# agnusmaximus/DistributedMNIST

Hardware: AMD Instinct MI355X
Metric: images/sec (whole node), MNIST CNN sync-SGD (higher is better)
Workload: dtype bf16; 1 GPU; model=lenet, global_batch=1024, parallelism=dp1, mode=full_sync, mode_requested=full_sync, grad_dtype=fp32

## Files before the change

csrc/bindings.cpp:

```cpp

#include <torch/extension.h>
#include <ATen/hip/HIPContext.h>
#include <hip/hip_runtime.h>

#include "kernels.h"

namespace {

#define CHECK_BF16(t) TORCH_CHECK((t).scalar_type() == at::kBFloat16, #t " must be bf16")
#define CHECK_F32(t) TORCH_CHECK((t).scalar_type() == at::kFloat, #t " must be fp32")
#define CHECK_CONTIG(t) TORCH_CHECK((t).is_contiguous(), #t " must be contiguous")
#define CHECK_CUDA(t) TORCH_CHECK((t).is_cuda(), #t " must be on GPU")

const unsigned short* bf16_ptr(const torch::Tensor& t) {
  return reinterpret_cast<const unsigned short*>(t.data_ptr());
}
unsigned short* bf16_mut(torch::Tensor& t) {
  return reinterpret_cast<unsigned short*>(t.data_ptr());
}

hipStream_t cur_stream() {
  return at::hip::getCurrentHIPStream().stream();
}

int cdiv(int a, int b) { return (a + b - 1) / b; }

int pick_splitk(int mtiles, int ntiles, int ksteps) {
  int tiles = mtiles * ntiles;
  if (tiles >= 256 || ksteps <= 1) return 1;
  int want = std::min(ksteps, std::max(1, 512 / tiles));
  return want;
}

int dw_tr_level() {
  static int v = [] {
    const char* e = getenv("DMNIST_DW_TR");
    return e ? atoi(e) : 1;
  }();
  return v;
}
bool dw_tr_enabled() { return dw_tr_level() != 0; }

torch::Tensor linear_act_fwd_impl(torch::Tensor x, torch::Tensor w,
                                  torch::Tensor b, bool relu, double p_keep,
                                  int64_t seed, int64_t offset,
                                  const long* offset_dev,
                                  const c10::optional<torch::Tensor>& wT) {
  CHECK_CUDA(x); CHECK_BF16(x); CHECK_CONTIG(x);
  CHECK_BF16(w); CHECK_CONTIG(w);
  CHECK_F32(b); CHECK_CONTIG(b);
  int M = x.size(0), K = x.size(1), N = w.size(1);
  TORCH_CHECK(w.size(0) == K, "w/x shape mismatch");
  auto y = torch::empty({M, N}, x.options());
  GemmParams p{};
  p.A = bf16_ptr(x);
  p.bias = b.data_ptr<float>();
  p.C = y.data_ptr(); p.amax = nullptr;
  p.M = M; p.N = N; p.K = K;
  p.lda = K; p.ldc = N;
  p.splitk = 1;
  p.p_keep = (float)p_keep; p.seed = (uint64_t)seed; p.offset = (uint64_t)offset;
  p.offset_dev = offset_dev;
  bool drop = p_keep < 1.0;
  TORCH_CHECK(!drop || relu, "dropout path requires relu epilogue");
  int g128 = cdiv(M, 128) * cdiv(N, 128);
  bool big = g128 >= 512;
  if (const char* e = getenv("DMNIST_FC_TILE")) big = atoi(e) >= 128;
  auto s = cur_stream();
  bool bt = wT.has_value() && wT->defined();
  int tiles64 = cdiv(M, 64) * cdiv(N, 64);
  int ksteps = cdiv(K, 64);
  if (!big && tiles64 < 256 && ksteps >= 16 &&
      !getenv("DMNIST_FC_NOSPLIT")) {
    int sk = std::min(ksteps, std::max(2, 512 / tiles64));
    auto acc = torch::empty({(int64_t)sk, (int64_t)M, (int64_t)N},
                            x.options().dtype(at::kFloat));
    p.C = acc.data_ptr();
    p.splitk = sk;
    if (bt) {
      CHECK_BF16((*wT)); CHECK_CONTIG((*wT));
      TORCH_CHECK(wT->size(0) == N && wT->size(1) == K, "wT shape mismatch");
      p.B = bf16_ptr(*wT); p.ldb = K;
      gemm_fwd_slices_64_bt(p, s);
    } else {
      p.B = bf16_ptr(w); p.ldb = N;
      gemm_fwd_slices_64(p, s);
    }
    launch_fwd_epilogue(acc.data_ptr<float>(), b.data_ptr<float>(),
                        bf16_mut(y), M, N, sk, relu ? 1 : 0, (float)p_keep,
                        (uint64_t)seed, (uint64_t)offset, offset_dev, s);
    return y;
  }
  if (bt) {
    CHECK_BF16((*wT)); CHECK_CONTIG((*wT));
    TORCH_CHECK(wT->size(0) == N && wT->size(1) == K, "wT shape mismatch");
    p.B = bf16_ptr(*wT); p.ldb = K;
    if (drop) (big ? gemm_fwd_drop_128_bt : gemm_fwd_drop_64_bt)(p, s);
    else if (relu) (big ? gemm_fwd_relu_128_bt : gemm_fwd_relu_64_bt)(p, s);
    else (big ? gemm_fwd_bias_128_bt : gemm_fwd_bias_64_bt)(p, s);
  } else {
    p.B = bf16_ptr(w); p.ldb = N;
    if (drop) (big ? gemm_fwd_drop_128 : gemm_fwd_drop_64)(p, s);
    else if (relu) (big ? gemm_fwd_relu_128 : gemm_fwd_relu_64)(p, s);
    else (big ? gemm_fwd_bias_128 : gemm_fwd_bias_64)(p, s);
  }
  return y;
}

torch::Tensor linear_act_fwd(torch::Tensor x, torch::Tensor w, torch::Tensor b,
                             bool relu, double p_keep, int64_t seed,
                             int64_t offset,
                             c10::optional<torch::Tensor> wT) {
  return linear_act_fwd_impl(x, w, b, relu, p_keep, seed, offset, nullptr, wT);
}

torch::Tensor linear_act_fwd_dev(torch::Tensor x, torch::Tensor w,
                                 torch::Tensor b, bool relu, double p_keep,
                                 int64_t seed, torch::Tensor offset_dev,
                                 c10::optional<torch::Tensor> wT) {
  TORCH_CHECK(offset_dev.scalar_type() == at::kLong && offset_dev.is_cuda(),
              "offset_dev must be a cuda int64 tensor");
  return linear_act_fwd_impl(x, w, b, relu, p_keep, seed, 0,
                             offset_dev.data_ptr<long>(), wT);
}

std::vector<torch::Tensor> linear_act_bwd_impl(torch::Tensor dy, torch::Tensor x,
                                               torch::Tensor w, torch::Tensor y,
                                               bool relu, double p_keep,
                                               bool need_dx,
                                               torch::Tensor dw, torch::Tensor db) {
  CHECK_CUDA(dy); CHECK_BF16(dy); CHECK_CONTIG(dy);
  CHECK_BF16(x); CHECK_CONTIG(x);
  CHECK_BF16(w); CHECK_CONTIG(w);
  int B = x.size(0), K = x.size(1), N = w.size(1);
  auto s = cur_stream();
  if (!db.defined())
    db = torch::zeros({N}, x.options().dtype(at::kFloat));
  CHECK_F32(db); CHECK_CONTIG(db);
  torch::Tensor dyeff;
  bool mask = relu || p_keep < 1.0;
  if (mask) {
    dyeff = torch::empty_like(dy);
    launch_relu_drop_bwd(bf16_ptr(dy), bf16_ptr(y), bf16_mut(dyeff),
                         db.data_ptr<float>(), B, N,
                         (float)(1.0 / p_keep), 1, s);
  } else {
    dyeff = dy;
    launch_relu_drop_bwd(bf16_ptr(dy), bf16_ptr(y), bf16_mut(dyeff),
                         db.data_ptr<float>(), B, N, 1.0f, 0, s);
  }
  if (!dw.defined())
    dw = torch::zeros({K, N}, x.options().dtype(at::kFloat));
  CHECK_F32(dw); CHECK_CONTIG(dw);
  {
    GemmParams p{};
    p.A = bf16_ptr(x); p.B = bf16_ptr(dyeff);
    p.C = dw.data_ptr();
    p.M = K; p.N = N; p.K = B;
    p.lda = K;
    p.ldb = N; p.ldc = N;
    if (dw_tr_enabled() && K % 8 == 0 && N % 64 == 0) {
      int bn = (N % 128 == 0) ? 128 : 64;
      p.splitk = pick_splitk(cdiv(K, 128), cdiv(N, bn), cdiv(B, 32));
      (bn == 128 ? gemm_dw_tr_128 : gemm_dw_tr_64)(p, s);
    } else {
      bool big = cdiv(K, 128) * cdiv(N, 128) >= 128;
      int bm = big ? 128 : 64;
      p.splitk = pick_splitk(cdiv(K, bm), cdiv(N, bm), cdiv(B, 32));
      (big ? gemm_dw_128 : gemm_dw_64)(p, s);
    }
  }
  torch::Tensor dx;
  if (need_dx) {
    dx = torch::empty({B, K}, x.options());
    GemmParams p{};
    p.A = bf16_ptr(dyeff); p.B = bf16_ptr(w);
    p.C = dx.data_ptr();
    p.M = B; p.N = K; p.K = N;
    p.lda = N; p.ldb = N; p.ldc = K;
    p.splitk = 1;
    bool big = cdiv(B, 128) * cdiv(K, 128) >= 128;
    (big ? gemm_dx_128 : gemm_dx_64)(p, s);
  } else {
    dx = torch::empty({0}, x.options());
  }
  return {dx, dw, db};
}

std::vector<torch::Tensor> linear_act_bwd(torch::Tensor dy, torch::Tensor x,
                                          torch::Tensor w, torch::Tensor y,
                                          bool relu, double p_keep,
                                          bool need_dx) {
  return linear_act_bwd_impl(dy, x, w, y, relu, p_keep, need_dx,
                             torch::Tensor(), torch::Tensor());
}

torch::Tensor linear_act_bwd_into(torch::Tensor dy, torch::Tensor x,
                                  torch::Tensor w, torch::Tensor y,
                                  bool relu, double p_keep, bool need_dx,
                                  torch::Tensor dw_out, torch::Tensor db_out) {
  auto r = linear_act_bwd_impl(dy, x, w, y, relu, p_keep, need_dx,
                               dw_out.view({x.size(1), w.size(1)}), db_out);
  return r[0];
}

std::vector<torch::Tensor> conv_pool_fwd(torch::Tensor x, torch::Tensor w,
                                         torch::Tensor b,
                                         c10::optional<torch::Tensor> wT) {
  CHECK_CUDA(x); CHECK_BF16(x); CHECK_CONTIG(x);
  CHECK_BF16(w); CHECK_CONTIG(w);
  CHECK_F32(b); CHECK_CONTIG(b);
  int NB = x.size(0), H = x.size(1), W = x.size(2), Cin = x.size(3);
  TORCH_CHECK(w.dim() == 4 && w.size(0) == 5 && w.size(1) == 5 &&
              w.size(2) == Cin, "conv weight must be [5,5,Cin,Cout]");
  int Cout = w.size(3);
  int Ho = H / 2, Wo = W / 2;
  auto y = torch::empty({NB, Ho, Wo, Cout}, x.options());
  auto amax = torch::empty({NB, Ho, Wo, Cout}, x.options().dtype(at::kByte));
  GemmParams p{};
  p.A = bf16_ptr(x); p.B = bf16_ptr(w);
  p.bias = b.data_ptr<float>();
  p.C = y.data_ptr(); p.amax = amax.data_ptr<uint8_t>();
  p.M = NB * Ho * Wo * 4; p.N = Cout; p.K = 25 * Cin;
  p.ldb = Cout; p.ldc = Cout;
  p.splitk = 1;
  p.CB = NB; p.CH = H; p.CW = W; p.CHo = Ho; p.CWo = Wo;
  p.Cin = Cin; p.Cout = Cout;
  auto s = cur_stream();
  if (Cin == 1 && conv1_mfma_supported(H, W, Cin, Cout) &&
      conv1_mfma_enabled() &&
      reinterpret_cast<uintptr_t>(x.data_ptr()) % 8 == 0) {
    launch_conv1_mfma_fwd(bf16_ptr(x), bf16_ptr(w), b.data_ptr<float>(),
                          bf16_mut(y), amax.data_ptr<uint8_t>(), NB, s);
  } else if (Cin == 1) {
    launch_conv1_direct_fwd(bf16_ptr(x), bf16_ptr(w), b.data_ptr<float>(),
                            bf16_mut(y), amax.data_ptr<uint8_t>(), NB, H, W,
                            Cout, s);
  } else if (conv_slab_supported(H, W, Cin, Cout)) {
    launch_conv_fwd_slab(bf16_ptr(x), bf16_ptr(w), b.data_ptr<float>(),
                         bf16_mut(y), amax.data_ptr<uint8_t>(), NB, H, W,
                         Cin, Cout, s);
  } else {
    TORCH_CHECK(Cin % 8 == 0, "conv requires Cin==1 or Cin%8==0");
    if (wT.has_value() && wT->defined()) {
      CHECK_BF16((*wT)); CHECK_CONTIG((*wT));
      p.B = bf16_ptr(*wT); p.ldb = 25 * Cin;
      conv_fwd_pool_bt(p, s);
    } else {
      conv_fwd_pool(p, s);
    }
  }
  return {y, amax};
}

std::vector<torch::Tensor> conv_pool_bwd_impl(torch::Tensor dy, torch::Tensor x,
                                              torch::Tensor w, torch::Tensor y,
                                              torch::Tensor amax, bool need_dx,
                                              torch::Tensor dw, torch::Tensor db) {
  CHECK_CUDA(dy); CHECK_BF16(dy); CHECK_CONTIG(dy);
  CHECK_BF16(x); CHECK_CONTIG(x); CHECK_BF16(w); CHECK_CONTIG(w);
  int NB = x.size(0), H = x.size(1), W = x.size(2), Cin = x.size(3);
  int Cout = w.size(3);
  int Ho = H / 2, Wo = W / 2;
  auto s = cur_stream();
  auto dact = torch::empty({NB, H, W, Cout}, x.options());
  if (!db.defined())
    db = torch::zeros({Cout}, x.options().dtype(at::kFloat));
  CHECK_F32(db); CHECK_CONTIG(db);
  launch_pool_bwd_scatter(bf16_ptr(dy), bf16_ptr(y),
                          amax.data_ptr<uint8_t>(), bf16_mut(dact),
                          db.data_ptr<float>(), NB * Ho * Wo, Cout, H, W, Wo,
                          s);
  if (!dw.defined())
    dw = torch::zeros({5, 5, Cin, Cout}, x.options().dtype(at::kFloat));
  CHECK_F32(dw); CHECK_CONTIG(dw);
  {
    GemmParams p{};
    p.A = bf16_ptr(x); p.B = bf16_ptr(dact);
    p.C = dw.data_ptr();
    p.M = 25 * Cin; p.N = Cout; p.K = NB * H * W;
    p.ldb = Cout; p.ldc = Cout;
    p.CB = NB; p.CH = H; p.CW = W; p.Cin = Cin; p.Cout = Cout;
    if (Cin == 1 && H <= 28 && W <= 28 && Cout <= 32 &&
        !getenv("DMNIST_DW1_SLAB")) {
      launch_conv1_dw_direct(bf16_ptr(x), bf16_ptr(dact),
                             dw.data_ptr<float>(), NB, H, W, Cout, s);
    } else if (Cin == 1 && conv1_slab_supported(H, W, Cin, Cout)) {
      launch_conv1_dw_slab(bf16_ptr(x), bf16_ptr(dact), dw.data_ptr<float>(),
                           NB, H, W, Cout, s);
    } else if (Cin == 1) {
      p.splitk = std::min(cdiv(p.K, 64), 2048);
      conv1_dw_gemm(p, s);
    } else if (conv_slab_supported(H, W, Cin, Cout) &&
               ((dw_tr_level() == 0 && NB >= 2048) || getenv("DMNIST_DW_G"))) {
      launch_conv_dw_slab(bf16_ptr(x), bf16_ptr(dact), dw.data_ptr<float>(),
                          NB, H, W, Cin, Cout, s);
    } else {
      int tiles = cdiv(p.M, 128) * cdiv(p.N, 64);
      int want = p.K <= 262144 ? 1024 : 2048;
      if (const char* e = getenv("DMNIST_DW_BLOCKS")) want = atoi(e);
      p.splitk = std::min(cdiv(p.K, 64), std::max(1, want / tiles));
      if (dw_tr_enabled() && Cin % 8 == 0 && Cout % 64 == 0)
        conv_dw_tr(p, s);
      else
        conv_dw_gemm(p, s);
    }
  }
  torch::Tensor dx;
  if (need_dx && conv_slab_supported(H, W, Cin, Cout)) {
    dx = torch::empty({NB, H, W, Cin}, x.options());
    launch_conv_dx_slab(bf16_ptr(dact), bf16_ptr(w), bf16_mut(dx), NB, H, W,
                        Cin, Cout, s);
  } else if (need_dx) {
    TORCH_CHECK(Cout % 32 == 0, "conv_dx requires Cout%32==0");
    dx = torch::empty({NB, H, W, Cin}, x.options());
    GemmParams p{};
    p.A = bf16_ptr(dact); p.B = bf16_ptr(w);
    p.C = dx.data_ptr();
    p.M = NB * H * W; p.N = Cin; p.K = 25 * Cout;
    p.ldc = Cin;
    p.CB = NB; p.CH = H; p.CW = W; p.Cin = Cin; p.Cout = Cout;
    p.splitk = 1;
    conv_dx_gemm(p, s);
  } else {
    dx = torch::empty({0}, x.options());
  }
  return {dx, dw, db};
}

std::vector<torch::Tensor> conv_pool_bwd(torch::Tensor dy, torch::Tensor x,
                                         torch::Tensor w, torch::Tensor y,
                                         torch::Tensor amax, bool need_dx) {
  return conv_pool_bwd_impl(dy, x, w, y, amax, need_dx, torch::Tensor(),
                            torch::Tensor());
}

torch::Tensor conv_pool_bwd_into(torch::Tensor dy, torch::Tensor x,
                                 torch::Tensor w, torch::Tensor y,
                                 torch::Tensor amax, bool need_dx,
                                 torch::Tensor dw_out, torch::Tensor db_out) {
  auto r = conv_pool_bwd_impl(dy, x, w, y, amax, need_dx,
                              dw_out.view_as(w), db_out);
  return r[0];
}

torch::Tensor mask_db(torch::Tensor dy, torch::Tensor y, bool relu,
                      double p_keep, torch::Tensor db_out) {
  CHECK_CUDA(dy); CHECK_BF16(dy); CHECK_CONTIG(dy);
  CHECK_F32(db_out); CHECK_CONTIG(db_out);
  int B = dy.size(0), N = dy.size(1);
  auto s = cur_stream();
  bool mask = relu || p_keep < 1.0;
  torch::Tensor dyeff = mask ? torch::empty_like(dy) : dy;
  launch_relu_drop_bwd(bf16_ptr(dy), mask ? bf16_ptr(y) : bf16_ptr(dy),
                       bf16_mut(dyeff), db_out.data_ptr<float>(), B, N,
                       (float)(1.0 / p_keep), mask ? 1 : 0, s);
  return dyeff;
}

void linear_dw_into(torch::Tensor x, torch::Tensor dyeff,
                    torch::Tensor dw_out) {
  CHECK_BF16(x); CHECK_CONTIG(x); CHECK_BF16(dyeff); CHECK_CONTIG(dyeff);
  CHECK_F32(dw_out);
  int B = x.size(0), K = x.size(1), N = dyeff.size(1);
  GemmParams p{};
  p.A = bf16_ptr(x); p.B = bf16_ptr(dyeff);
  p.C = dw_out.data_ptr();
  p.M = K; p.N = N; p.K = B;
  p.lda = K; p.ldb = N; p.ldc = N;
  if (dw_tr_enabled() && K % 8 == 0 && N % 64 == 0) {
    int bn = (N % 128 == 0) ? 128 : 64;
    p.splitk = pick_splitk(cdiv(K, 128), cdiv(N, bn), cdiv(B, 32));
    (bn == 128 ? gemm_dw_tr_128 : gemm_dw_tr_64)(p, cur_stream());
    return;
  }
  bool big = cdiv(K, 128) * cdiv(N, 128) >= 128;
  int bm = big ? 128 : 64;
  p.splitk = pick_splitk(cdiv(K, bm), cdiv(N, bm), cdiv(B, 32));
  (big ? gemm_dw_128 : gemm_dw_64)(p, cur_stream());
}

torch::Tensor linear_dx(torch::Tensor dyeff, torch::Tensor w) {
  CHECK_BF16(dyeff); CHECK_CONTIG(dyeff); CHECK_BF16(w); CHECK_CONTIG(w);
  int B = dyeff.size(0), N = dyeff.size(1), K = w.size(0);
  auto dx = torch::empty({B, K}, dyeff.options());
  GemmParams p{};
  p.A = bf16_ptr(dyeff); p.B = bf16_ptr(w);
  p.C = dx.data_ptr();
  p.M = B; p.N = K; p.K = N;
  p.lda = N; p.ldb = N; p.ldc = K;
  p.splitk = 1;
  bool big = cdiv(B, 128) * cdiv(K, 128) >= 128;
  (big ? gemm_dx_128 : gemm_dx_64)(p, cur_stream());
  return dx;
}

torch::Tensor linear_dx_unpool(torch::Tensor dyeff, torch::Tensor w,
                               torch::Tensor amax, torch::Tensor db_out,
                               int64_t Ho, int64_t Wo, int64_t C) {
  CHECK_BF16(dyeff); CHECK_CONTIG(dyeff); CHECK_BF16(w); CHECK_CONTIG(w);
  int B = dyeff.size(0), N = dyeff.size(1), K = w.size(0);
  TORCH_CHECK(K == Ho * Wo * C, "linear_dx_unpool: K != Ho*Wo*C");
  auto dact = torch::empty({B, 2 * (int)Ho, 2 * (int)Wo, (int)C},
                           dyeff.options());
  GemmParams p{};
  p.A = bf16_ptr(dyeff); p.B = bf16_ptr(w);
  p.C = dact.data_ptr();
  p.M = B; p.N = K; p.K = N;
  p.lda = N; p.ldb = N; p.ldc = K;
  p.splitk = 1;
  p.CHo = Ho; p.CWo = Wo; p.Cout = C;
  p.amax = amax.data_ptr<uint8_t>();
  p.db = db_out.defined() ? db_out.data_ptr<float>() : nullptr;
  bool big = cdiv(B, 128) * cdiv(K, 128) >= 512;
  (big ? gemm_dx_unpool_128 : gemm_dx_unpool_64)(p, cur_stream());
  return dact;
}

torch::Tensor linear_dx_mask(torch::Tensor dyeff, torch::Tensor w,
                             torch::Tensor actm, torch::Tensor db_out,
                             double p_keep) {
  CHECK_BF16(dyeff); CHECK_CONTIG(dyeff); CHECK_BF16(w); CHECK_CONTIG(w);
  CHECK_BF16(actm); CHECK_CONTIG(actm);
  int B = dyeff.size(0), N = dyeff.size(1), K = w.size(0);
  TORCH_CHECK(actm.size(0) == B && actm.size(1) == K, "actm shape mismatch");
  auto dx = torch::empty({B, K}, dyeff.options());
  GemmParams p{};
  p.A = bf16_ptr(dyeff); p.B = bf16_ptr(w);
  p.C = dx.data_ptr();
  p.M = B; p.N = K; p.K = N;
  p.lda = N; p.ldb = N; p.ldc = K;
  p.splitk = 1;
  p.p_keep = (float)(1.0 / p_keep);
  p.actm = bf16_ptr(actm);
  p.db = db_out.defined() ? db_out.data_ptr<float>() : nullptr;
  bool big = cdiv(B, 128) * cdiv(K, 128) >= 128;
  (big ? gemm_dx_mask_128 : gemm_dx_mask_64)(p, cur_stream());
  return dx;
}

torch::Tensor pool_scatter(torch::Tensor dy, torch::Tensor y,
                           torch::Tensor amax, torch::Tensor db_out,
                           int64_t H, int64_t W) {
  CHECK_BF16(dy); CHECK_CONTIG(dy);
  int NB = dy.size(0), Ho = dy.size(1), Wo = dy.size(2), C = dy.size(3);
  auto dact = torch::empty({NB, (int)H, (int)W, C}, dy.options());
  launch_pool_bwd_scatter(bf16_ptr(dy), bf16_ptr(y),
                          amax.data_ptr<uint8_t>(), bf16_mut(dact),
                          db_out.data_ptr<float>(), NB * Ho * Wo, C, H, W,
                          Wo, cur_stream());
  return dact;
}

void conv_dw_into(torch::Tensor x, torch::Tensor dact, torch::Tensor dw_out) {
  CHECK_BF16(x); CHECK_CONTIG(x); CHECK_BF16(dact); CHECK_CONTIG(dact);
  int NB = x.size(0), H = x.size(1), W = x.size(2), Cin = x.size(3);
  int Cout = dact.size(3);
  auto s = cur_stream();
  GemmParams p{};
  p.A = bf16_ptr(x); p.B = bf16_ptr(dact);
  p.C = dw_out.data_ptr();
  p.M = 25 * Cin; p.N = Cout; p.K = NB * H * W;
  p.ldb = Cout; p.ldc = Cout;
  p.CB = NB; p.CH = H; p.CW = W; p.Cin = Cin; p.Cout = Cout;
  if (Cin == 1 && H <= 28 && W <= 28 && Cout <= 32 &&
      !getenv("DMNIST_DW1_SLAB")) {
    launch_conv1_dw_direct(bf16_ptr(x), bf16_ptr(dact),
                           dw_out.data_ptr<float>(), NB, H, W, Cout, s);
  } else if (Cin == 1 && conv1_slab_supported(H, W, Cin, Cout)) {
    launch_conv1_dw_slab(bf16_ptr(x), bf16_ptr(dact),
                         dw_out.data_ptr<float>(), NB, H, W, Cout, s);
  } else if (Cin == 1) {
    p.splitk = std::min(cdiv(p.K, 64), 2048);
    conv1_dw_gemm(p, s);
  } else if (conv_slab_supported(H, W, Cin, Cout) &&
             ((dw_tr_level() == 0 && NB >= 2048) || getenv("DMNIST_DW_G"))) {
    launch_conv_dw_slab(bf16_ptr(x), bf16_ptr(dact), dw_out.data_ptr<float>(),
                        NB, H, W, Cin, Cout, s);
  } else {
    int tiles = cdiv(p.M, 128) * cdiv(p.N, 64);
    int want = p.K <= 262144 ? 1024 : 2048;
    if (const char* e = getenv("DMNIST_DW_BLOCKS")) want = atoi(e);
    p.splitk = std::min(cdiv(p.K, 64), std::max(1, want / tiles));
    if (getenv("DMNIST_DW_SPREAD")) {
      static torch::Tensor scratch;
      int64_t need = 16LL * p.M * p.N;
      if (!scratch.defined() || scratch.numel() < need)
        scratch = torch::zeros({need}, dact.options().dtype(at::kFloat));
      p.C = scratch.data_ptr();
      p.offset = 1;
    }
    if (dw_tr_enabled() && Cin % 8 == 0 && Cout % 64 == 0)
      conv_dw_tr(p, s);
    else
      conv_dw_gemm(p, s);
  }
}

void conv1_dw_pooled(torch::Tensor x, torch::Tensor dyp, torch::Tensor am,
                     torch::Tensor dw_out, torch::Tensor db_out) {
  CHECK_BF16(x); CHECK_CONTIG(x);
  CHECK_BF16(dyp); CHECK_CONTIG(dyp);
  int NB = x.size(0), H = x.size(1), W = x.size(2);
  int Cout = dyp.size(3);
  TORCH_CHECK(x.size(3) == 1 && H == 28 && W == 28 && Cout == 32 &&
                  dyp.size(1) == H / 2 && dyp.size(2) == W / 2,
              "conv1_dw_pooled: LeNet conv1 shapes only");
  CHECK_CONTIG(am); CHECK_F32(dw_out); CHECK_CONTIG(dw_out);
  if (conv1_mfma_supported(H, W, 1, Cout) && conv1_mfma_enabled() &&
      reinterpret_cast<uintptr_t>(x.data_ptr()) % 8 == 0) {
    launch_conv1_mfma_dw(bf16_ptr(x), bf16_ptr(dyp), am.data_ptr<uint8_t>(),
                         dw_out.data_ptr<float>(),
                         db_out.defined() ? db_out.data_ptr<float>() : nullptr,
                         NB, cur_stream());
    return;
  }
  launch_conv1_dw_pooled(bf16_ptr(x), bf16_ptr(dyp),
                         am.data_ptr<uint8_t>(), dw_out.data_ptr<float>(),
                         db_out.defined() ? db_out.data_ptr<float>() : nullptr,
                         NB, H, W, Cout, cur_stream());
}

torch::Tensor conv_dx(torch::Tensor dact, torch::Tensor w, int64_t Cin) {
  CHECK_BF16(dact); CHECK_CONTIG(dact); CHECK_BF16(w); CHECK_CONTIG(w);
  int NB = dact.size(0), H = dact.size(1), W = dact.size(2),
      Cout = dact.size(3);
  auto s = cur_stream();
  auto dx = torch::empty({NB, H, W, (int)Cin}, dact.options());
  if (conv_slab_supported(H, W, Cin, Cout)) {
    launch_conv_dx_slab(bf16_ptr(dact), bf16_ptr(w), bf16_mut(dx), NB, H, W,
                        Cin, Cout, s);
  } else {
    TORCH_CHECK(Cout % 32 == 0, "conv_dx requires Cout%32==0");
    GemmParams p{};
    p.A = bf16_ptr(dact); p.B = bf16_ptr(w);
    p.C = dx.data_ptr();
    p.M = NB * H * W; p.N = Cin; p.K = 25 * Cout;
    p.ldc = Cin;
    p.CB = NB; p.CH = H; p.CW = W; p.Cin = Cin; p.Cout = Cout;
    p.splitk = 1;
    conv_dx_gemm(p, s);
  }
  return dx;
}

std::vector<torch::Tensor> softmax_xent_fwd(torch::Tensor logits,
                                            torch::Tensor labels,
                                            c10::optional<torch::Tensor> db_out,
                                            double inv_n) {
  CHECK_CUDA(logits); CHECK_BF16(logits); CHECK_CONTIG(logits);
  TORCH_CHECK(labels.scalar_type() == at::kLong, "labels must be int64");
  CHECK_CONTIG(labels);
  int B = logits.size(0), C = logits.size(1);
  TORCH_CHECK(C <= 16, "softmax_xent kernel supports C<=16");
  TORCH_CHECK(B <= 256 * SOFTMAX_MAX_BLOCKS, "softmax_xent: batch too large");
  auto dl = torch::empty_like(logits);
  auto out = torch::empty({2}, logits.options().dtype(at::kFloat));
  static std::vector<torch::Tensor>* ws = new std::vector<torch::Tensor>(64);
  int dev = logits.get_device();
  TORCH_CHECK(dev >= 0 && dev < 64, "softmax_xent: bad device index");
  if (!(*ws)[dev].defined()) {
    hipStreamCaptureStatus cap = hipStreamCaptureStatusNone;
    hipStreamIsCapturing(cur_stream(), &cap);
    TORCH_CHECK(cap == hipStreamCaptureStatusNone,
                "softmax_xent_fwd: first call on a device allocates its "
                "workspace and must run outside graph capture");
    (*ws)[dev] = torch::zeros({2 * SOFTMAX_MAX_BLOCKS + 1},
                              logits.options().dtype(at::kFloat));
  }
  float* part = (*ws)[dev].data_ptr<float>();
  unsigned* ticket = reinterpret_cast<unsigned*>(part + 2 * SOFTMAX_MAX_BLOCKS);
  float* dbp = nullptr;
  if (db_out.has_value() && db_out->defined())
    dbp = db_out->data_ptr<float>();
  launch_softmax_xent(bf16_ptr(logits), labels.data_ptr<long>(),
                      bf16_mut(dl), out.data_ptr<float>(), B, C, dbp,
                      (float)inv_n, part, ticket, cur_stream());
  auto loss = out.select(0, 0);
  auto correct = out.select(0, 1);
  return {loss, correct, dl};
}

void sgd_step(torch::Tensor master, torch::Tensor grad, torch::Tensor shadow,
              bool has_shadow, double lr, double scale, double dc_keep,
              int64_t seed, int64_t offset,
              c10::optional<torch::Tensor> momentum, double mu) {
  CHECK_CUDA(master); CHECK_F32(master); CHECK_CONTIG(master);
  CHECK_F32(grad); CHECK_CONTIG(grad);
  float* mom = nullptr;
  if (momentum.has_value() && momentum->defined()) {
    CHECK_F32((*momentum)); CHECK_CONTIG((*momentum));
    mom = momentum->data_ptr<float>();
  }
  launch_sgd_step(master.data_ptr<float>(), grad.data_ptr<float>(),
                  has_shadow ? bf16_mut(shadow) : nullptr,
                  has_shadow ? 1 : 0, master.numel(),
                  (float)(lr * scale), (float)dc_keep, (uint64_t)seed,
                  (uint64_t)offset, mom, (float)mu, cur_stream());
}

void sgd_step_dev(torch::Tensor master, torch::Tensor grad,
                  torch::Tensor shadow, bool has_shadow,
                  torch::Tensor lr_scale_dev, double dc_keep, int64_t seed,
                  torch::Tensor offset_dev,
                  c10::optional<torch::Tensor> momentum, double mu,
                  bool zero_grad) {
  CHECK_CUDA(master); CHECK_F32(master); CHECK_CONTIG(master);
  CHECK_F32(grad); CHECK_CONTIG(grad);
  CHECK_F32(lr_scale_dev);
  float* mom = nullptr;
  if (momentum.has_value() && momentum->defined()) {
    CHECK_F32((*momentum)); CHECK_CONTIG((*momentum));
    mom = momentum->data_ptr<float>();
  }
  launch_sgd_step_dev(master.data_ptr<float>(), grad.data_ptr<float>(),
                      has_shadow ? bf16_mut(shadow) : nullptr,
                      has_shadow ? 1 : 0, master.numel(),
                      lr_scale_dev.data_ptr<float>(), (float)dc_keep,
                      (uint64_t)seed, offset_dev.data_ptr<long>(),
                      mom, (float)mu, zero_grad ? 1 : 0, cur_stream());
}

void transpose_bf16_batch(std::vector<torch::Tensor> srcs,
                          std::vector<torch::Tensor> dsts) {
  TORCH_CHECK(srcs.size() == dsts.size() && srcs.size() <= 4,
              "up to 4 transpose pairs");
  TransposeDesc d[4];
  for (size_t i = 0; i < srcs.size(); ++i) {
    CHECK_BF16(srcs[i]); CHECK_CONTIG(srcs[i]);
    CHECK_BF16(dsts[i]); CHECK_CONTIG(dsts[i]);
    d[i] = {bf16_ptr(srcs[i]), bf16_mut(dsts[i]),
            (int)srcs[i].size(0), (int)srcs[i].size(1)};
  }
  launch_transpose_bf16_batch(d, (int)srcs.size(), cur_stream());
}

void transpose_bf16_batch_adv(std::vector<torch::Tensor> srcs,
                              std::vector<torch::Tensor> dsts,
                              torch::Tensor step_dev,
                              torch::Tensor lr_scale_dev, double lr0,
                              double decay, int64_t decay_steps,
                              double inv_contrib) {
  TORCH_CHECK(srcs.size() == dsts.size() && srcs.size() <= 4,
              "up to 4 transpose pairs");
  TransposeDesc d[4];
  for (size_t i = 0; i < srcs.size(); ++i) {
    CHECK_BF16(srcs[i]); CHECK_CONTIG(srcs[i]);
    CHECK_BF16(dsts[i]); CHECK_CONTIG(dsts[i]);
    d[i] = {bf16_ptr(srcs[i]), bf16_mut(dsts[i]),
            (int)srcs[i].size(0), (int)srcs[i].size(1)};
  }
  launch_transpose_bf16_batch_adv(
      d, (int)srcs.size(), step_dev.data_ptr<long>(),
      lr_scale_dev.data_ptr<float>(), (float)lr0, (float)decay,
      (int)decay_steps, (float)inv_contrib, cur_stream());
}

void transpose_bf16(torch::Tensor src, torch::Tensor dst) {
  CHECK_CUDA(src); CHECK_BF16(src); CHECK_CONTIG(src);
  CHECK_BF16(dst); CHECK_CONTIG(dst);
  TORCH_CHECK(src.dim() == 2 && dst.size(0) == src.size(1) &&
              dst.size(1) == src.size(0), "transpose shape mismatch");
  launch_transpose_bf16(bf16_ptr(src), bf16_mut(dst), src.size(0),
                        src.size(1), cur_stream());
}

void step_advance(torch::Tensor step_dev, torch::Tensor lr_scale_dev,
                  double lr0, double decay, int64_t decay_steps,
                  double inv_contrib) {
  launch_step_advance(step_dev.data_ptr<long>(),
                      lr_scale_dev.data_ptr<float>(), (float)lr0,
                      (float)decay, (int)decay_steps, (float)inv_contrib,
                      cur_stream());
}

void grad_mask(torch::Tensor g, double keep, int64_t seed, int64_t step,
               int64_t rank, int64_t base,
               c10::optional<torch::Tensor> step_dev) {
  CHECK_CUDA(g); CHECK_F32(g); CHECK_CONTIG(g);
  TORCH_CHECK(base % 4 == 0,
              "grad_mask: slice base must be 16B-aligned so slice-wise "
              "masks compose to the whole-buffer mask");
  const long* sd = nullptr;
  if (step_dev.has_value() && step_dev->defined())
    sd = step_dev->data_ptr<long>();
  launch_grad_mask(g.data_ptr<float>(), g.numel(), base, (float)keep,
                   (uint64_t)seed, (uint64_t)step, (uint64_t)rank, sd,
                   cur_stream());
}

void batch_gather(torch::Tensor img_u8, torch::Tensor lab_u8,
                  torch::Tensor lut, torch::Tensor x, torch::Tensor y,
                  int64_t seed, int64_t step,
                  c10::optional<torch::Tensor> step_dev) {
  CHECK_CUDA(img_u8); CHECK_CONTIG(img_u8);
  CHECK_CUDA(lab_u8); CHECK_CONTIG(lab_u8);
  CHECK_CUDA(lut); CHECK_BF16(lut); CHECK_CONTIG(lut);
  CHECK_CUDA(x); CHECK_BF16(x); CHECK_CONTIG(x);
  CHECK_CUDA(y); CHECK_CONTIG(y);
  TORCH_CHECK(img_u8.scalar_type() == at::kByte &&
              lab_u8.scalar_type() == at::kByte,
              "batch_gather: images/labels must be uint8");
  TORCH_CHECK(y.scalar_type() == at::kLong, "batch_gather: y must be int64");
  const int64_t N = lab_u8.numel(), B = y.numel();
  TORCH_CHECK(N >= 1 && N < (int64_t(1) << 31),
              "batch_gather: N out of range");
  TORCH_CHECK(B >= 1 && B <= N, "batch_gather: batch size ", B,
              " must be in [1, N=", N, "]");
  TORCH_CHECK(img_u8.numel() == N * 784, "batch_gather: images must be [N,784]");
  TORCH_CHECK(x.numel() == B * 784, "batch_gather: x must hold B*784 values");
  TORCH_CHECK(lut.numel() == 256, "batch_gather: lut must have 256 entries");
  TORCH_CHECK(reinterpret_cast<uintptr_t>(img_u8.data_ptr()) % 8 == 0 &&
              reinterpret_cast<uintptr_t>(x.data_ptr()) % 16 == 0,
              "batch_gather: images must be 8B- and x 16B-aligned");
  const long* sd = nullptr;
  if (step_dev.has_value() && step_dev->defined()) {
    TORCH_CHECK(step_dev->is_cuda() && step_dev->scalar_type() == at::kLong &&
                step_dev->numel() >= 1, "batch_gather: step_dev must be a "
                "device int64 tensor");
    sd = step_dev->data_ptr<long>();
  } else {
    TORCH_CHECK(step >= 0, "batch_gather: step must be >= 0");
  }
  launch_batch_gather(img_u8.data_ptr<uint8_t>(), lab_u8.data_ptr<uint8_t>(),
                      bf16_ptr(lut), bf16_mut(x), y.data_ptr<long>(),
                      (uint32_t)N, (uint32_t)B, (uint64_t)seed,
                      (uint64_t)step, sd, cur_stream());
}

}

PYBIND11_MODULE(TORCH_EXTENSION_NAME, m) {
  m.def("linear_act_fwd", &linear_act_fwd, "fused linear+bias+relu+dropout",
        py::arg("x"), py::arg("w"), py::arg("b"), py::arg("relu"),
        py::arg("p_keep"), py::arg("seed"), py::arg("offset"),
        py::arg("wT") = c10::nullopt);
  m.def("transpose_bf16", &transpose_bf16, "bf16 2-D transpose (wT refresh)");
  m.def("transpose_bf16_batch_adv", &transpose_bf16_batch_adv,
        "batched transposes + fused device step/LR advance (graph tail)");
  m.def("transpose_bf16_batch", &transpose_bf16_batch,
        "up to 4 transposes in one launch");
  m.def("mask_db", &mask_db, "relu/dropout grad mask + bias-grad column sums");
  m.def("linear_dw_into", &linear_dw_into, "dW = x^T dyeff into bucket view");
  m.def("linear_dx", &linear_dx, "dx = dyeff @ W^T");
  m.def("linear_dx_mask", &linear_dx_mask,
        "dx GEMM with fused relu/dropout mask + bias-grad column sums",
        py::arg("dyeff"), py::arg("w"), py::arg("actm"), py::arg("db_out"),
        py::arg("p_keep"));
  m.def("linear_dx_unpool", &linear_dx_unpool,
        "dx GEMM fused with maxpool2x2 backward scatter + conv db",
        py::arg("dyeff"), py::arg("w"), py::arg("amax"),
        py::arg("db_out"), py::arg("Ho"), py::arg("Wo"), py::arg("C"));
  m.def("pool_scatter", &pool_scatter, "maxpool bwd scatter + conv db");
  m.def("conv_dw_into", &conv_dw_into, "conv dW into bucket view");
  m.def("conv1_dw_pooled", &conv1_dw_pooled,
        "conv1 dW+db from the pooled gradient (pool bwd fused, no dact1)",
        py::arg("x"), py::arg("dyp"), py::arg("am"),
        py::arg("dw_out"), py::arg("db_out"));
  m.def("conv1_dw_group", [](int64_t NB) {
          return (int64_t)conv1_mfma_dw_group((int)NB);
        }, "images per block the MFMA conv1 dW launcher picks for batch NB");
  m.def("conv_dx", &conv_dx, "conv dX");
  m.def("linear_act_bwd", &linear_act_bwd, "linear backward (dx, dw, db)");
  m.def("linear_act_bwd_into", &linear_act_bwd_into,
        "linear backward accumulating dw/db into bucket views");
  m.def("conv_pool_fwd", &conv_pool_fwd, "fused conv5x5+bias+relu+maxpool",
        py::arg("x"), py::arg("w"), py::arg("b"), py::arg("wT") = c10::nullopt);
  m.def("conv_pool_bwd", &conv_pool_bwd, "conv+pool backward (dx, dw, db)");
  m.def("conv_pool_bwd_into", &conv_pool_bwd_into,
        "conv backward accumulating dw/db into bucket views");
  m.def("softmax_xent_fwd", &softmax_xent_fwd, "fused softmax-CE (+grad, +optional fc2 db, +optional acc-mean scale)",
        py::arg("logits"), py::arg("labels"),
        py::arg("db_out") = c10::nullopt, py::arg("inv_n") = 1.0);
  m.def("sgd_step", &sgd_step, "fused flat SGD(+momentum) apply",
        py::arg("master"), py::arg("grad"), py::arg("shadow"),
        py::arg("has_shadow"), py::arg("lr"), py::arg("scale"),
        py::arg("dc_keep"), py::arg("seed"), py::arg("offset"),
        py::arg("momentum") = c10::nullopt, py::arg("mu") = 0.0);
  m.def("sgd_step_dev", &sgd_step_dev,
        "SGD apply with device-side lr/offset (hipGraph-capturable); "
        "zero_grad clears the bucket in the same pass",
        py::arg("master"), py::arg("grad"), py::arg("shadow"),
        py::arg("has_shadow"), py::arg("lr_scale_dev"), py::arg("dc_keep"),
        py::arg("seed"), py::arg("offset_dev"),
        py::arg("momentum") = c10::nullopt, py::arg("mu") = 0.0,
        py::arg("zero_grad") = false);
  m.def("step_advance", &step_advance,
        "device-side staircase LR + step increment (inside the graph)");
  m.def("grad_mask", &grad_mask,
        "per-rank pre-aggregation drop-connect mask (in-place, philox; "
        "reference distributed_train.py:194-203)",
        py::arg("g"), py::arg("keep"), py::arg("seed"), py::arg("step"),
        py::arg("rank"), py::arg("base") = 0,
        py::arg("step_dev") = c10::nullopt);
  m.def("batch_gather", &batch_gather,
        "gather one training batch from the device-resident uint8 set "
        "(Feistel epoch permutation keyed on seed + step; LUT-normalised "
        "to bf16) into x [B,28,28,1] bf16 / y [B] int64",
        py::arg("img_u8"), py::arg("lab_u8"), py::arg("lut"), py::arg("x"),
        py::arg("y"), py::arg("seed"), py::arg("step"),
        py::arg("step_dev") = c10::nullopt);
  m.def("linear_act_fwd_dev", &linear_act_fwd_dev,
        "linear fwd with device-side dropout offset",
        py::arg("x"), py::arg("w"), py::arg("b"), py::arg("relu"),
        py::arg("p_keep"), py::arg("seed"), py::arg("offset_dev"),
        py::arg("wT") = c10::nullopt);
}
```

csrc/build.py:

```python
#!/usr/bin/env python3

import os
import subprocess
import sys
import sysconfig

ROOT = os.path.dirname(os.path.abspath(__file__))


def main():
    import torch
    import torch.utils.cpp_extension as ce

    torch_inc = ce.include_paths()
    torch_lib = ce.library_paths()[0]
    py_inc = sysconfig.get_paths()["include"]
    hipcc = os.environ.get("HIPCC", "/opt/rocm/bin/hipcc")
    abi = int(torch.compiled_with_cxx11_abi())

    srcs = [os.path.join(ROOT, f) for f in
            ("gemm_tile.hip", "conv_slab.hip", "dw_tr.hip", "ops_misc.hip", "conv1_mfma.hip",
             "data_gather.hip",
             "bindings.cpp")]
    out = os.path.join(ROOT, "_dmnist_hip.so")

    cmd = [hipcc, "--offload-arch=gfx950", "-O3", "-std=c++17", "-fPIC",
           "-shared", "-x", "hip"] + srcs + [
        "-o", out,
        f"-D_GLIBCXX_USE_CXX11_ABI={abi}",
        "-DTORCH_EXTENSION_NAME=_dmnist_hip",
        "-DTORCH_API_INCLUDE_EXTENSION_H",
        "-DUSE_ROCM=1", "-D__HIP_PLATFORM_AMD__=1",
        "-DHIP_ENABLE_WARP_SYNC_BUILTINS=1",
        "-fno-gpu-rdc",
        "-Wno-deprecated-declarations",
    ]
    cmd += [f"-I{p}" for p in torch_inc + [py_inc, ROOT]]
    cmd += [f"-L{torch_lib}", "-ltorch", "-ltorch_cpu", "-ltorch_hip",
            "-lc10", "-lc10_hip", "-ltorch_python",
            "-L/opt/rocm/lib", "-lamdhip64",
            f"-Wl,-rpath,{torch_lib}", "-Wl,-rpath,/opt/rocm/lib"]
    print("[build]", " ".join(cmd), flush=True)
    subprocess.run(cmd, check=True)
    print(f"[build] wrote {out}")


if __name__ == "__main__":
    main()
```

csrc/kernels.h:

```cpp
#pragma once
#include <hip/hip_runtime.h>
#include <stdint.h>

struct GemmParams {
  const unsigned short* A;
  const unsigned short* B;
  const float* bias;
  void* C;
  uint8_t* amax;
  int M, N, K;
  int lda, ldb, ldc;
  int splitk;
  int CB, CH, CW, CHo, CWo, Cin, Cout;
  float p_keep;
  uint64_t seed, offset;
  const long* offset_dev;
  float* db;
  const unsigned short* actm;
};

void gemm_fwd_bias_128(const GemmParams&, hipStream_t);
void gemm_fwd_bias_64(const GemmParams&, hipStream_t);
void gemm_fwd_relu_128(const GemmParams&, hipStream_t);
void gemm_fwd_relu_64(const GemmParams&, hipStream_t);
void gemm_fwd_drop_128(const GemmParams&, hipStream_t);
void gemm_fwd_drop_64(const GemmParams&, hipStream_t);
void gemm_dx_128(const GemmParams&, hipStream_t);
void gemm_dx_64(const GemmParams&, hipStream_t);
void gemm_dx_unpool_128(const GemmParams&, hipStream_t);
void gemm_dx_unpool_64(const GemmParams&, hipStream_t);
void gemm_dx_mask_128(const GemmParams&, hipStream_t);
void gemm_dx_mask_64(const GemmParams&, hipStream_t);
void gemm_dw_128(const GemmParams&, hipStream_t);
void gemm_dw_64(const GemmParams&, hipStream_t);
void conv_fwd_pool(const GemmParams&, hipStream_t);
void conv1_fwd_pool(const GemmParams&, hipStream_t);
void conv_dx_gemm(const GemmParams&, hipStream_t);
void conv_dw_gemm(const GemmParams&, hipStream_t);
void conv_dw_tr(const GemmParams&, hipStream_t);
void gemm_dw_tr_128(const GemmParams&, hipStream_t);
void gemm_dw_tr_64(const GemmParams&, hipStream_t);

void launch_relu_drop_bwd(const unsigned short* dy, const unsigned short* y,
                          unsigned short* dyeff, float* db, int B, int N,
                          float inv_keep, int apply_mask, hipStream_t);
void launch_pool_bwd_scatter(const unsigned short* dy, const unsigned short* y,
                             const uint8_t* amax, unsigned short* dact,
                             float* db, int Mpool, int C, int H, int W, int Wo,
                             hipStream_t);
#define SOFTMAX_MAX_BLOCKS 4096
void launch_softmax_xent(const unsigned short* logits, const long* labels,
                         unsigned short* dlogits, float* out, int B, int C,
                         float* db, float inv_n, float* part,
                         unsigned* ticket, hipStream_t);
void launch_sgd_step(float* master, float* grad, unsigned short* shadow,
                     int has_shadow, long n, float lr_scale, float dc_keep,
                     uint64_t seed, uint64_t offset, float* momentum, float mu,
                     hipStream_t);
void launch_sgd_step_dev(float* master, float* grad,
                         unsigned short* shadow, int has_shadow, long n,
                         const float* lr_scale_dev, float dc_keep,
                         uint64_t seed, const long* offset_dev,
                         float* momentum, float mu, int zero_grad,
                         hipStream_t);
void launch_conv1_dw_pooled(const unsigned short* x, const unsigned short* dyp,
                            const uint8_t* am, float* dw, float* db, int NB,
                            int H, int W, int Cout, hipStream_t s);
void launch_grad_mask(float* g, long n, long base, float keep, uint64_t seed,
                      uint64_t step, uint64_t rank, const long* step_dev,
                      hipStream_t s);
void launch_step_advance(long* step_dev, float* lr_scale_dev, float lr0,
                         float decay, int decay_steps, float inv_contrib,
                         hipStream_t);
void launch_batch_gather(const uint8_t* img, const uint8_t* lab,
                         const unsigned short* lut, unsigned short* x,
                         long* y, uint32_t N, uint32_t B, uint64_t seed,
                         uint64_t step, const long* step_dev, hipStream_t);
void launch_transpose_bf16(const unsigned short* src, unsigned short* dst,
                           int R, int C, hipStream_t);
struct TransposeDesc {
  const unsigned short* src;
  unsigned short* dst;
  int R, C;
};
struct TransposeBatchArgs {
  TransposeDesc d[4];
  int tile0[4];
  int n, total;
  int do_advance;
  long* step_dev;
  float* lr_scale_dev;
  float lr0, decay, inv_contrib;
  int decay_steps;
};
void launch_transpose_bf16_batch(const TransposeDesc* descs, int n,
                                 hipStream_t);
void launch_transpose_bf16_batch_adv(const TransposeDesc* descs, int n,
                                     long* step_dev, float* lr_scale_dev,
                                     float lr0, float decay, int decay_steps,
                                     float inv_contrib, hipStream_t);
void launch_conv1_direct_fwd(const unsigned short* x, const unsigned short* w,
                             const float* bias, unsigned short* y,
                             uint8_t* amax, int NB, int H, int W, int Cout,
                             hipStream_t);
void gemm_fwd_bias_128_bt(const GemmParams&, hipStream_t);
void gemm_fwd_bias_64_bt(const GemmParams&, hipStream_t);
void gemm_fwd_relu_128_bt(const GemmParams&, hipStream_t);
void gemm_fwd_relu_64_bt(const GemmParams&, hipStream_t);
void gemm_fwd_drop_128_bt(const GemmParams&, hipStream_t);
void gemm_fwd_drop_64_bt(const GemmParams&, hipStream_t);
void conv_fwd_pool_bt(const GemmParams&, hipStream_t);
void conv1_dw_gemm(const GemmParams&, hipStream_t);
bool conv_slab_supported(int H, int W, int Cin, int Cout);
void launch_conv_fwd_slab(const unsigned short* x, const unsigned short* w,
                          const float* bias, unsigned short* y, uint8_t* amax,
                          int NB, int H, int W, int Cin, int Cout, hipStream_t);
void launch_conv_dx_slab(const unsigned short* dact, const unsigned short* w,
                         unsigned short* dx, int NB, int H, int W, int Cin,
                         int Cout, hipStream_t);
void launch_conv_dw_slab(const unsigned short* x, const unsigned short* dact,
                         float* dw, int NB, int H, int W, int Cin, int Cout,
                         hipStream_t);
bool conv1_slab_supported(int H, int W, int Cin, int Cout);
void launch_conv1_dw_slab(const unsigned short* x, const unsigned short* dact,
                          float* dw, int NB, int H, int W, int Cout,
                          hipStream_t);
void launch_conv1_dw_direct(const unsigned short* x,
                            const unsigned short* dact, float* dw, int NB,
                            int H, int W, int Cout, hipStream_t s);
bool conv1_mfma_supported(int H, int W, int Cin, int Cout);
bool conv1_mfma_enabled();
int conv1_mfma_dw_group(int NB);
void launch_conv1_mfma_fwd(const unsigned short* x, const unsigned short* w,
                           const float* bias, unsigned short* y,
                           uint8_t* amax, int NB, hipStream_t);
void launch_conv1_mfma_dw(const unsigned short* x, const unsigned short* dyp,
                          const uint8_t* am, float* dw, float* db, int NB,
                          hipStream_t);
void gemm_fwd_slices_64(const GemmParams&, hipStream_t);
void gemm_fwd_slices_64_bt(const GemmParams&, hipStream_t);
void launch_fwd_epilogue(const float* acc, const float* bias,
                         unsigned short* y, int M, int N, int slices,
                         int relu, float p_keep, uint64_t seed,
                         uint64_t offset, const long* offset_dev,
                         hipStream_t);
```

Baseline: 3.372 million images/sec.

## Add specialized slab MFMA kernel for conv2 weight gradient

Adds a dedicated conv2 (14x14, 32->64) dW kernel that stages each image's input rows and output gradient into LDS through direct global-to-LDS loads. It then accumulates all 5x5 taps with bf16 MFMA and transposed LDS reads, split per kernel row across blocks, and finally atomically adds into the fp32 dW. The kernel is routed by default in place of the generic transposed split-K GEMM path. The aim is to cut im2col-style redundant loads and split-K overhead, at the cost of atomics and extra code specialized to one shape.

```diff
diff --git a/csrc/bindings.cpp b/csrc/bindings.cpp
--- a/csrc/bindings.cpp
+++ b/csrc/bindings.cpp
@@ -40,6 +40,11 @@
   return v;
 }
 bool dw_tr_enabled() { return dw_tr_level() != 0; }
+
+bool conv2_dw_slab_route(int H, int W, int Cin, int Cout) {
+  return conv2_dw_slab_supported(H, W, Cin, Cout) && dw_tr_enabled() &&
+         conv2_dw_slab_enabled() && !getenv("DMNIST_DW_SPREAD");
+}
 
 torch::Tensor linear_act_fwd_impl(torch::Tensor x, torch::Tensor w,
                                   torch::Tensor b, bool relu, double p_keep,
@@ -295,6 +300,9 @@
                ((dw_tr_level() == 0 && NB >= 2048) || getenv("DMNIST_DW_G"))) {
       launch_conv_dw_slab(bf16_ptr(x), bf16_ptr(dact), dw.data_ptr<float>(),
                           NB, H, W, Cin, Cout, s);
+    } else if (conv2_dw_slab_route(H, W, Cin, Cout)) {
+      launch_conv2_dw_slab(bf16_ptr(x), bf16_ptr(dact), dw.data_ptr<float>(),
+                           NB, s);
     } else {
       int tiles = cdiv(p.M, 128) * cdiv(p.N, 64);
       int want = p.K <= 262144 ? 1024 : 2048;
@@ -477,6 +485,9 @@
              ((dw_tr_level() == 0 && NB >= 2048) || getenv("DMNIST_DW_G"))) {
     launch_conv_dw_slab(bf16_ptr(x), bf16_ptr(dact), dw_out.data_ptr<float>(),
                         NB, H, W, Cin, Cout, s);
+  } else if (conv2_dw_slab_route(H, W, Cin, Cout)) {
+    launch_conv2_dw_slab(bf16_ptr(x), bf16_ptr(dact),
+                         dw_out.data_ptr<float>(), NB, s);
   } else {
     int tiles = cdiv(p.M, 128) * cdiv(p.N, 64);
     int want = p.K <= 262144 ? 1024 : 2048;
@@ -760,6 +771,9 @@
   m.def("conv1_dw_group", [](int64_t NB) {
           return (int64_t)conv1_mfma_dw_group((int)NB);
         }, "images per block the MFMA conv1 dW launcher picks for batch NB");
+  m.def("conv2_dw_group", [](int64_t NB) {
+          return (int64_t)conv2_dw_group((int)NB);
+        }, "images per block the slab conv2 dW launcher picks for batch NB");
   m.def("conv_dx", &conv_dx, "conv dX");
   m.def("linear_act_bwd", &linear_act_bwd, "linear backward (dx, dw, db)");
   m.def("linear_act_bwd_into", &linear_act_bwd_into,
diff --git a/csrc/build.py b/csrc/build.py
--- a/csrc/build.py
+++ b/csrc/build.py
@@ -20,7 +20,7 @@
 
     srcs = [os.path.join(ROOT, f) for f in
             ("gemm_tile.hip", "conv_slab.hip", "dw_tr.hip", "ops_misc.hip", "conv1_mfma.hip",
-             "data_gather.hip",
+             "data_gather.hip", "conv2_dw_slab.hip",
              "bindings.cpp")]
     out = os.path.join(ROOT, "_dmnist_hip.so")
 
diff --git a/csrc/conv2_dw_slab.hip b/csrc/conv2_dw_slab.hip
--- /dev/null
+++ b/csrc/conv2_dw_slab.hip
@@ -0,0 +1,220 @@
+
+#include "common.h"
+#include "kernels.h"
+#include <stdlib.h>
+#include <stdexcept>
+
+#define C2_MG 8
+#define C2_XIMG (14 * 14 * 32)
+#define C2_DIMG (14 * 14 * 64)
+
+static __device__ __align__(16) unsigned short c2_zero_page[8];
+
+DEV int c2_xswz(int s) { return ((s >> 3) & 1) << 1; }
+DEV int c2_dswz(int k) { return (((k >> 1) & 1) | (((k >> 3) & 1) << 1)) << 1; }
+
+extern __shared__ __align__(16) ushort_t c2_lds[];
+
+template <int KHB, int NBUF>
+__global__ __launch_bounds__(256, (KHB == 1 && NBUF == 1) ? 3 : 1)
+void conv2_dw_slab_kernel(const ushort_t* __restrict__ x,
+                          const ushort_t* __restrict__ dact,
+                          float* __restrict__ dw, int NB, int G) {
+  constexpr int NRX = 13 + KHB;
+  constexpr int XPIX = C2_MG + NRX * 16 + C2_MG;
+  constexpr int NJOB = NRX + 28;
+  constexpr int NQ = (NJOB + 3) / 4;
+  constexpr int NKB = 5 / KHB;
+  constexpr int KS_UNROLL = KHB == 1 ? 7 : 1;
+  constexpr int BUF = XPIX * 32 + 224 * 64;
+  ushort_t* const X = c2_lds;
+  ushort_t* const D = c2_lds + XPIX * 32;
+
+  const int tid = threadIdx.x;
+  const int lane = tid & 63, wave = tid >> 6;
+  const int wr = wave >> 1, wc = wave & 1;
+
+  const int pos = blockIdx.x >> 3;
+  const int grp = (pos / NKB) * 8 + (blockIdx.x & 7);
+  const int kh0 = (pos % NKB) * KHB;
+  const int img0 = grp * G;
+  if (img0 >= NB) return;
+
+  if (tid < 64 * NBUF) {
+    int t = tid & 63;
+    int o = (t < 32) ? t * 8 : (C2_MG + NRX * 16) * 32 + (t - 32) * 8;
+    *reinterpret_cast<short8*>(X + (tid >> 6) * BUF + o) =
+        short8{0, 0, 0, 0, 0, 0, 0, 0};
+  }
+
+  int soff[NQ];
+#pragma unroll
+  for (int q = 0; q < NQ; ++q) {
+    int j = wave + 4 * q;
+    soff[q] = -1;
+    if (j < NRX) {
+      int ir = j + kh0 - 2, px = lane >> 2;
+      int lc = (lane & 3) ^ c2_xswz(C2_MG + j * 16 + px);
+      if (px < 14 && ir >= 0 && ir < 14) soff[q] = (ir * 14 + px) * 32 + lc * 8;
+    } else if (j < NJOB) {
+      int jj = j - NRX;
+      int h = jj >> 1, px = (jj & 1) * 8 + (lane >> 3);
+      int lc = (lane & 7) ^ c2_dswz(h * 16 + px);
+      if (px < 14) soff[q] = (h * 14 + px) * 64 + lc * 8;
+    }
+  }
+  const auto issue = [&](int buf, int img) {
+    const ushort_t* xi = x + (size_t)img * C2_XIMG;
+    const ushort_t* di = dact + (size_t)img * C2_DIMG;
+#pragma unroll
+    for (int q = 0; q < NQ; ++q) {
+      int j = wave + 4 * q;
+      if (j < NRX) {
+        const ushort_t* src = soff[q] >= 0 ? xi + soff[q] : c2_zero_page;
+        glds16(src, X + buf * BUF + (C2_MG + j * 16) * 32);
+      } else if (j < NJOB) {
+        const ushort_t* src = soff[q] >= 0 ? di + soff[q] : c2_zero_page;
+        glds16(src, D + buf * BUF + (j - NRX) * 8 * 64);
+      }
+    }
+  };
+
+  const int r0 = (lane >> 4) * 8 + ((lane & 15) >> 2);
+  const int cp = (lane & 3) >> 1, off8 = (lane & 1) * 8;
+  unsigned aaddr[5][2], baddr[2][2];
+#pragma unroll
+  for (int kw = 0; kw < 5; ++kw)
+#pragma unroll
+    for (int t = 0; t < 2; ++t) {
+      int s = C2_MG + r0 + 4 * t + kw - 2;
+      aaddr[kw][t] = (unsigned)(uintptr_t)X +
+                     (unsigned)(s * 64 + (((wr * 2 + cp) ^ c2_xswz(s)) << 4) +
+                                off8);
+    }
+#pragma unroll
+  for (int ni = 0; ni < 2; ++ni)
+#pragma unroll
+    for (int t = 0; t < 2; ++t) {
+      int k = r0 + 4 * t;
+      baddr[ni][t] = (unsigned)(uintptr_t)D +
+                     (unsigned)(k * 128 +
+                                (((wc * 4 + ni * 2 + cp) ^ c2_dswz(k)) << 4) +
+                                off8);
+    }
+
+  f32x4 acc[KHB][5][2];
+#pragma unroll
+  for (int a = 0; a < KHB; ++a)
+#pragma unroll
+    for (int b = 0; b < 5; ++b)
+#pragma unroll
+      for (int c = 0; c < 2; ++c) acc[a][b][c] = f32x4{0.f, 0.f, 0.f, 0.f};
+
+  const int n = min(G, NB - img0);
+  if (NBUF == 2) issue(0, img0);
+  for (int g = 0; g < n; ++g) {
+    if (NBUF == 1) {
+      __syncthreads();
+      issue(0, img0 + g);
+    }
+    asm volatile("s_waitcnt vmcnt(0)" ::: "memory");
+    __syncthreads();
+    if (NBUF == 2 && g + 1 < n) issue((g + 1) & 1, img0 + g + 1);
+    const unsigned boff = (unsigned)((g & (NBUF - 1)) * BUF * 2);
+#pragma unroll KS_UNROLL
+    for (int ks = 0; ks < 7; ++ks) {
+      uint2 br[2][2];
+#pragma unroll
+      for (int ni = 0; ni < 2; ++ni)
+#pragma unroll
+        for (int t = 0; t < 2; ++t)
+          br[ni][t] = tr16_issue(baddr[ni][t] + boff + ks * (32 * 128));
+#pragma unroll
+      for (int khl = 0; khl < KHB; ++khl) {
+        uint2 ar[5][2];
+#pragma unroll
+        for (int kw = 0; kw < 5; ++kw)
+#pragma unroll
+          for (int t = 0; t < 2; ++t)
+            ar[kw][t] = tr16_issue(aaddr[kw][t] + boff +
+                                   (ks * 32 + khl * 16) * 64);
+        short8 af[5], bf[2];
+#pragma unroll
+        for (int kw = 0; kw < 5; ++kw) af[kw] = pack_wait(ar[kw][0], ar[kw][1]);
+#pragma unroll
+        for (int ni = 0; ni < 2; ++ni) bf[ni] = pack_wait(br[ni][0], br[ni][1]);
+#pragma unroll
+        for (int kw = 0; kw < 5; ++kw)
+#pragma unroll
+          for (int ni = 0; ni < 2; ++ni)
+            acc[khl][kw][ni] = __builtin_amdgcn_mfma_f32_16x16x32_bf16(
+                af[kw], bf[ni], acc[khl][kw][ni], 0, 0, 0);
+      }
+    }
+  }
+
+  const int frow = (lane >> 4) * 4, fcol = lane & 15;
+#pragma unroll
+  for (int khl = 0; khl < KHB; ++khl)
+#pragma unroll
+    for (int kw = 0; kw < 5; ++kw)
+#pragma unroll
+      for (int ni = 0; ni < 2; ++ni)
+#pragma unroll
+        for (int r = 0; r < 4; ++r) {
+          int m = ((kh0 + khl) * 5 + kw) * 32 + wr * 16 + frow + r;
+          int n = wc * 32 + ni * 16 + fcol;
+          atomicAdd(dw + m * 64 + n, acc[khl][kw][ni][r]);
+        }
+}
+
+
+bool conv2_dw_slab_supported(int H, int W, int Cin, int Cout) {
+  return H == 14 && W == 14 && Cin == 32 && Cout == 64;
+}
+
+bool conv2_dw_slab_enabled() {
+  const char* e = getenv("DMNIST_DW2_SLAB");
+  return !(e && atoi(e) == 0);
+}
+
+int conv2_dw_group(int NB) {
+  int G = NB >= 4096 ? 32 : (NB >= 512 ? 12 : (NB >= 128 ? 4 : 1));
+  if (const char* e = getenv("DMNIST_DW2_G")) G = atoi(e);
+  return G < 1 ? 1 : G;
+}
+
+template <int KHB, int NBUF>
+static void c2_launch(const unsigned short* x, const unsigned short* dact,
+                      float* dw, int NB, int G, int blocks, hipStream_t s) {
+  constexpr int BYTES = NBUF * ((C2_MG * 2 + (13 + KHB) * 16) * 32 + 224 * 64) * 2;
+  if (BYTES > 65536) {
+    static const hipError_t granted = hipFuncSetAttribute(
+        reinterpret_cast<const void*>(&conv2_dw_slab_kernel<KHB, NBUF>),
+        hipFuncAttributeMaxDynamicSharedMemorySize, BYTES);
+    if (granted != hipSuccess)
+      throw std::runtime_error("conv2_dw_slab: LDS size not granted");
+  }
+  hipLaunchKernelGGL((conv2_dw_slab_kernel<KHB, NBUF>), dim3(blocks),
+                     dim3(256), BYTES, s, x, dact, dw, NB, G);
+}
+
+void launch_conv2_dw_slab(const unsigned short* x, const unsigned short* dact,
+                          float* dw, int NB, hipStream_t s) {
+  if (NB <= 0) return;
+  int G = conv2_dw_group(NB);
+  int groups = (NB + G - 1) / G;
+  int g8 = (groups + 7) / 8 * 8;
+  const char* e = getenv("DMNIST_DW2_KHB");
+  const char* b = getenv("DMNIST_DW2_NBUF");
+  bool all_taps = e && atoi(e) == 5;
+  int nbuf = b ? atoi(b) : 1;
+  if (all_taps && nbuf == 2)
+    c2_launch<5, 2>(x, dact, dw, NB, G, g8, s);
+  else if (all_taps)
+    c2_launch<5, 1>(x, dact, dw, NB, G, g8, s);
+  else if (nbuf == 2)
+    c2_launch<1, 2>(x, dact, dw, NB, G, g8 * 5, s);
+  else
+    c2_launch<1, 1>(x, dact, dw, NB, G, g8 * 5, s);
+}
diff --git a/csrc/kernels.h b/csrc/kernels.h
--- a/csrc/kernels.h
+++ b/csrc/kernels.h
@@ -137,6 +137,11 @@
 void launch_conv1_mfma_dw(const unsigned short* x, const unsigned short* dyp,
                           const uint8_t* am, float* dw, float* db, int NB,
                           hipStream_t);
+bool conv2_dw_slab_supported(int H, int W, int Cin, int Cout);
+bool conv2_dw_slab_enabled();
+int conv2_dw_group(int NB);
+void launch_conv2_dw_slab(const unsigned short* x, const unsigned short* dact,
+                          float* dw, int NB, hipStream_t);
 void gemm_fwd_slices_64(const GemmParams&, hipStream_t);
 void gemm_fwd_slices_64_bt(const GemmParams&, hipStream_t);
 void launch_fwd_epilogue(const float* acc, const float* bias,
```

Result: faster. 3.619 million images/sec, median of 6 (+7.3%).
